# shionhonda/gae-dgl

Hardware: AMD Instinct MI355X
Metric: edges aggregated/sec (SpMM fwd+bwd) (higher is better)
Workload: dtype f32 (storage, aggregations, accumulators; the dense products run on the 16-bit matrix pipe from split operands with fp32 accumulation: X W^T and dW from three bf16 pieces per operand / six pairs, the loss from two fp16 pieces (N >= 5120) or three bf16 pieces -- all fp32-grade, see ms_per_step_exact_

## Files before the change

gae_dgl_amd/csrc/common.h:

```cpp
#pragma once
#include <hip/hip_runtime.h>
#include <stdint.h>
#include <stdio.h>

#include <atomic>

#include "gae_hip.h"
#include "gae_hip_experimental.h"

namespace gae {

struct Knob {
    std::atomic<int> v;
    explicit constexpr Knob(int x) : v(x) {}
    operator int() const { return v.load(std::memory_order_relaxed); }
    Knob &operator=(int x) { v.store(x, std::memory_order_relaxed); return *this; }
};

extern Knob g_spmm_variant, g_spmm_rpg, g_spmm_tile_vecs, g_spmm_ell, g_spmm_ell_rpg, g_spmm_hot, g_spmm_desc, g_spmm_light;
extern Knob g_gemm_rows, g_linear_wlds, g_atb_bf16, g_ell_side;
extern Knob g_xw_rows, g_xw_parts, g_xw_glds, g_xw_p3;
extern Knob g_bce_s_bf16, g_bce_pv_bf16, g_bce_sym, g_bce_sym_ri, g_bce_sym_bal, g_bce_last_kind;
extern Knob g_topk_splits, g_rank_splits;

// ... 38 lines not shown
    const unsigned xcd = bid % kNumXcd, k = bid / kNumXcd;
    const unsigned base = xcd < r ? xcd * (q + 1) : r * (q + 1) + (xcd - r) * q;
    return base + k;
}

__device__ __forceinline__ float bf16_to_f32(unsigned short v)
{
    return __uint_as_float(static_cast<unsigned>(v) << 16);
}
__device__ __forceinline__ unsigned short f32_to_bf16(float f)
{
    unsigned u = __float_as_uint(f);
    if ((u & 0x7fffffffu) > 0x7f800000u) return static_cast<unsigned short>((u >> 16) | 0x40);
    u += 0x7fffu + ((u >> 16) & 1u);
    return static_cast<unsigned short>(u >> 16);
}

typedef float v4f __attribute__((ext_vector_type(4)));
typedef float v2f __attribute__((ext_vector_type(2)));
typedef short v4s __attribute__((ext_vector_type(4)));
typedef int v4i __attribute__((ext_vector_type(4)));
typedef __bf16 v2bf __attribute__((ext_vector_type(2)));

__device__ __forceinline__ void split_bf16x4(const v4f &v, v4s &hi, v4s &lo)
{
    unsigned h[2], l[2];
#pragma unroll
    for (int q = 0; q < 2; ++q) {
        const v2f a = {v[2 * q], v[2 * q + 1]};
        const unsigned hu = __builtin_bit_cast(unsigned, __builtin_convertvector(a, v2bf));
// ... 86 lines not shown
```

gae_dgl_amd/csrc/decoder_bce.hip:

```cpp
#include <string.h>

#include "common.h"
#include "bce_finalize.h"

namespace {

using gae::kWave;
typedef float f32x4 __attribute__((ext_vector_type(4)));
typedef short s16x4 __attribute__((ext_vector_type(4)));
typedef float f32x2 __attribute__((ext_vector_type(2)));
typedef __bf16 bf16x2 __attribute__((ext_vector_type(2)));

constexpr int TJ = 64;
constexpr int PREP_ROWS = 64;
constexpr int kBceRi = 2;
constexpr int64_t kBceGrid = 2048;
constexpr int64_t kBceSymGrid = 16384;
constexpr int kChipCus = 256;
}

namespace gae {
Knob g_bce_s_bf16{3};
Knob g_bce_last_kind{0};
Knob g_bce_sym_bal{1};
// ... 43 lines not shown
    asm("v_fma_f32 %0, %1, %2, -0.5" : "=v"(s1) : "v"(r01), "v"(t[0]));
    asm("v_fma_f32 %0, %1, %2, -0.5" : "=v"(s2) : "v"(r23), "v"(t[3]));
    asm("v_fma_f32 %0, %1, %2, -0.5" : "=v"(s3) : "v"(r23), "v"(t[2]));
    return f32x4{copysignf(s0, y[0]), copysignf(s1, y[1]), copysignf(s2, y[2]), copysignf(s3, y[3])};
}

__global__ __launch_bounds__(256) void bce_prepare_kernel(const float *__restrict__ Z, float *__restrict__ mask,
                                                          int64_t ldz, int64_t n, int d, int DP, int64_t row_begin,
                                                          int64_t row_end, float *__restrict__ Zt,
                                                          unsigned short *__restrict__ Zhi,
                                                          unsigned short *__restrict__ Zlo,
                                                          double *__restrict__ colsum_partial ,
                                                          float drop_p, float drop_scale, uint64_t seed,
                                                          uint64_t offset, const uint64_t *__restrict__ draw_dev,
                                                          const int64_t *__restrict__ counts ,
                                                          double *__restrict__ scal , double all_pairs)
{
    __shared__ double red[2][256];
    const int tid = threadIdx.x;
    const int64_t n_valid = counts ? counts[0] : n;
    if (counts && blockIdx.x == 0 && tid == 0) {
        const double nv = double(counts[0]), ev = double(counts[1]);
        scal[0] = ev > 0 ? (nv * nv - ev) / ev : 0.0;
        scal[1] = nv > 0 ? 1.0 / (nv * nv) : 0.0;
        scal[2] = all_pairs - nv * nv;
    }
    const int k = tid % DP, rl = tid / DP, rpp = 256 / DP;
    const int64_t r0 = int64_t(blockIdx.x) * PREP_ROWS;
    double s_all = 0.0, s_win = 0.0;
    const bool draw = drop_p > 0.f;
    const uint64_t draw_idx = (draw && draw_dev) ? *draw_dev : 0;
    for (int rr = rl; rr < PREP_ROWS; rr += rpp) {
        const int64_t i = r0 + rr;
        if (i >= n) break;
        float v = 0.f;
        if (k < d && i >= n_valid) {
            if (draw) mask[i * ldz + k] = 0.f;
        } else if (k < d) {
            v = Z[i * ldz + k];
            if (draw) {
                const int64_t e = i * d + k;
                uint32_t c[4];
                gae::philox4x32_10(offset + uint64_t(e >> 2), draw_idx, seed, c);
                const uint32_t bits = (e & 2) ? ((e & 1) ? c[3] : c[2]) : ((e & 1) ? c[1] : c[0]);
                const float m = gae::dropout_multiplier(bits, drop_p, drop_scale);
                mask[i * ldz + k] = m;
                v *= m;
            } else if (mask) {
                v *= mask[i * ldz + k];
            }
        }
        Zt[i * DP + k] = v;
        const unsigned short hi = gae::f32_to_bf16(v);
        Zhi[i * DP + k] = hi;
        Zlo[i * DP + k] = gae::f32_to_bf16(v - gae::bf16_to_f32(hi));
        s_all += double(v);
        if (i >= row_begin && i < row_end) s_win += double(v);
    }
    red[0][tid] = s_all; red[1][tid] = s_win;
    __syncthreads();
    if (tid < DP) {
        double a = 0.0, w = 0.0;
        for (int q = 0; q < rpp; ++q) { a += red[0][q * DP + tid]; w += red[1][q * DP + tid]; }
        colsum_partial[(int64_t(blockIdx.x) * 2 + 0) * DP + tid] = a;
        colsum_partial[(int64_t(blockIdx.x) * 2 + 1) * DP + tid] = w;
    }
}

__device__ __forceinline__ void bce_colsum_block(const double *__restrict__ colsum_partial, int64_t n_blocks, int DP,
                                                 double *__restrict__ S ,
                                                 float *__restrict__ S_all_f , double *red )
{
    const int k = threadIdx.x % DP, q = threadIdx.x / DP, nq = 256 / DP;
// ... 76 lines not shown
    unsigned l2[2];
#pragma unroll
    for (int q = 0; q < 2; ++q) {
        const f32x2 a = {v[2 * q], v[2 * q + 1]};
        const f32x2 fh = {gae::bf16_to_f32((unsigned short)hi[2 * q]), gae::bf16_to_f32((unsigned short)hi[2 * q + 1])};
        const f32x2 fl = {gae::bf16_to_f32((unsigned short)lo[2 * q]), gae::bf16_to_f32((unsigned short)lo[2 * q + 1])};
        l2[q] = __builtin_bit_cast(unsigned, __builtin_convertvector((a - fh) - fl, bf16x2));
    }
    struct U { unsigned a, b; } u{l2[0], l2[1]};
    return __builtin_bit_cast(s16x4, u);
}

typedef _Float16 f16x8 __attribute__((ext_vector_type(8)));
typedef _Float16 f16x4 __attribute__((ext_vector_type(4)));
typedef __fp16 fp16x2 __attribute__((ext_vector_type(2)));
constexpr float kF16Max = 32768.f;
__device__ __forceinline__ f32x4 mfma32h(const s16x8 &a, const s16x8 &b, const f32x4 &c)
{
    return __builtin_amdgcn_mfma_f32_16x16x32_f16(__builtin_bit_cast(f16x8, a), __builtin_bit_cast(f16x8, b), c, 0, 0, 0);
}
template <bool F16>
__device__ __forceinline__ f32x4 mfma_k32(const s16x8 &a, const s16x8 &b, const f32x4 &c)
{
    if constexpr (F16) return mfma32h(a, b, c);
    else return mfma32(a, b, c);
}
typedef _Float16 f16x2 __attribute__((ext_vector_type(2)));
__device__ __forceinline__ float minus_f16_lo(float v, unsigned hh)
{
    float r;
    asm("v_fma_mix_f32 %0, %1, -1.0, %2 op_sel_hi:[1,0,0]" : "=v"(r) : "v"(hh), "v"(v));
// ... 487 lines not shown
    ew.start(Zt, DP, i, i, rowv, f0, true, wk.indptr, wk.t_indptr);
    double lsum = ew.run(Zt, DP, f0, true, pw, wk.indices, wk.t_indices);
    if (rowv) {
        f32x4 v;
#pragma unroll
        for (int q = 0; q < 4; ++q) v[q] = ew.acc_in[q] + ew.acc_out[q];
        *reinterpret_cast<f32x4 *>(wk.s + i * DP + f0) = v;
    }
#pragma unroll
    for (int off = 32; off > 0; off >>= 1) lsum += __shfl_down(lsum, off, 64);
    if (lane == 0) red[wave][0] = lsum;
    __syncthreads();
    if (tid == 0) wk.loss_partial[w] = (red[0][0] + red[1][0]) + (red[2][0] + red[3][0]);
}

enum class SymForm { kF16, kBf16x3, kBf16x3Fallback };

template <bool WITH_GRAD, int RI, SymForm FORM, bool BAL>
__global__ __launch_bounds__(256, (RI == 2 && FORM != SymForm::kBf16x3Fallback) ? 3 : 2) void bce_dense_sym_kernel(
    const float *__restrict__ Zt , const unsigned short *__restrict__ Zhi,
    const unsigned short *__restrict__ Zlo, int64_t n, int64_t cols_per_chunk,
    float *__restrict__ O_partial , float *__restrict__ Wmir,
    double *__restrict__ loss_partial , const double *__restrict__ colsum_partial,
    int64_t n_prep_blocks, double *__restrict__ S, float *__restrict__ S_all_f, unsigned n_panels, int exp_strip,
    unsigned *__restrict__ range_flag, int flag_mode, unsigned ticket, unsigned n_chunks, int bal_tpb,
    const SymWalkArgs wk)
{
    if (flag_mode == 2 && *range_flag != ticket) return;
    constexpr bool F16 = FORM == SymForm::kF16;
    constexpr bool PERSIST = FORM == SymForm::kBf16x3Fallback;
    bool out_of_range = false;
    constexpr int DP = 16, SYM_PR = 64 * RI;
    constexpr int LDH = DP + 4;
    constexpr int V4 = TJ * DP / 4 / 256;
    constexpr int LDM = TJ + 4;
    constexpr int LDHL = 2 * DP + 8;
    __shared__ __attribute__((aligned(16))) unsigned short HLs[2][TJ * LDHL];
    __shared__ __attribute__((aligned(16))) unsigned short L2s[2][F16 ? 4 : TJ * LDH];
    __shared__ __attribute__((aligned(16))) float MR[2][4][16 * LDM];
    __shared__ double red[4][2];

  double sumA = 0.0, sumL = 0.0;
  auto unit = [&](const int64_t I, const int64_t col_begin, const int64_t col_end, const int64_t op_slot, const int64_t lp_index) {
    const int tid = threadIdx.x, lane = tid & 63, wave = tid >> 6;
    const int l15 = lane & 15, g = lane >> 4;
    const int64_t NP = (n + 63) / 64 * 64;
    const int64_t row_base = SYM_PR * I + wave * (RI * 16);
    const int64_t diag_end = SYM_PR * (I + 1);

    constexpr float LOG2E = 1.44269504088896341f;
    static_assert(RI % 2 == 0, "row subtiles are paired into K = 32 mirror products");
    s16x8 bhh[RI];
    s16x8 bll[RI];
    s16x8 b3[F16 ? 1 : RI];
    s16x8 zTh[RI / 2], zTl[RI / 2];
#pragma unroll
    for (int ri = 0; ri < RI; ++ri) {
        const int64_t i = row_base + ri * 16 + l15;
        f32x4 b = *reinterpret_cast<const f32x4 *>(Zt + (i < n ? i : 0) * DP + 4 * g);
        if (i >= n) b = f32x4{0.f, 0.f, 0.f, 0.f};
        b *= LOG2E;
        s16x4 bhi, blo, blo2;
        if (F16) {
            out_of_range |= !(fmaxf(fmaxf(fabsf(b[0]), fabsf(b[1])), fmaxf(fabsf(b[2]), fabsf(b[3]))) <= kF16Max * LOG2E);
            split_f16x4(b, bhi, blo);
        } else {
            split_bf16x4_3(b, bhi, blo, blo2);
            b3[ri] = cat(bhi, blo2);
        }
        bhh[ri] = cat(bhi, bhi);
        bll[ri] = cat(blo, blo);
        s16x4 th, tl;
#pragma unroll
        for (int r = 0; r < 4; ++r) {
            const int64_t ir = row_base + ri * 16 + 4 * g + r;
            const bool v = ir < n;
            if (F16) continue;
            th[r] = v ? short(Zhi[(v ? ir : 0) * DP + l15]) : short(0);
            tl[r] = v ? short(Zlo[(v ? ir : 0) * DP + l15]) : short(0);
// ... 37 lines not shown
            const int jj = idx / (DP / 4), kk = (idx % (DP / 4)) * 4;
            const bool jv = j0 + jj < col_end;
            const int64_t j = jv ? j0 + jj : col_begin;
            st.f[q] = *reinterpret_cast<const f32x4 *>(Zt + j * DP + kk);
            if (!jv) st.f[q] = f32x4{0.f, 0.f, 0.f, 0.f};
        }
    };
    auto store_tile = [&](int buf, const Stage &st) {
#pragma unroll
        for (int q = 0; q < V4; ++q) {
            const int idx = tid + 256 * q;
            const int jj = idx / (DP / 4), kk = (idx % (DP / 4)) * 4;
            s16x4 h4, l4;
            if (F16) {
                const f32x4 f = st.f[q];
                out_of_range |= !(fmaxf(fmaxf(fabsf(f[0]), fabsf(f[1])), fmaxf(fabsf(f[2]), fabsf(f[3]))) <= kF16Max);
                split_f16x4(f, h4, l4);
            } else {
                s16x4 l24;
                split_bf16x4_3(st.f[q], h4, l4, l24);
                *reinterpret_cast<s16x4 *>(&L2s[buf][jj * LDH + kk]) = l24;
            }
            *reinterpret_cast<s16x8 *>(&HLs[buf][jj * LDHL + 2 * kk]) = cat(h4, l4);
        }
    };
    float *strip = Wmir + sym_strip_offset(I, NP, SYM_PR);
    auto flush_mirror = [&](int64_t j0, int mb) {
        const int f = tid >> 4, jq = (tid & 15) * 4;
        f32x4 v = *reinterpret_cast<const f32x4 *>(&MR[mb][0][f * LDM + jq]);
#pragma unroll
        for (int w = 1; w < 4; ++w) v += *reinterpret_cast<const f32x4 *>(&MR[mb][w][f * LDM + jq]);
// ... 106 lines not shown
        compute_tile(buf, j0, offdiag);
        if (more) store_tile(buf ^ 1, stage);
        __syncthreads();
        if (WITH_GRAD && offdiag) flush_mirror(j0, buf);
    }
    if (WITH_GRAD) {
        float *op = O_partial + op_slot * n * DP;
#pragma unroll
        for (int ri = 0; ri < RI; ++ri)
#pragma unroll
            for (int r = 0; r < 4; ++r) {
                const int64_t i = row_base + ri * 16 + 4 * g + r;
                if (i < n) op[i * DP + l15] = oacc[ri][r];
            }
    }
    if (F16 && flag_mode == 1 && out_of_range) atomicExch(range_flag, ticket);
    if (BAL) return;
    double la = sumA * 0.69314718055994531, ll = sumL;
#pragma unroll
    for (int off = 32; off > 0; off >>= 1) { la += __shfl_down(la, off, 64); ll += __shfl_down(ll, off, 64); }
    if (lane == 0) { red[wave][0] = la; red[wave][1] = ll; }
    __syncthreads();
    if (tid == 0) {
        loss_partial[2 * lp_index + 0] = (red[0][0] + red[1][0]) + (red[2][0] + red[3][0]);
        loss_partial[2 * lp_index + 1] = (red[0][1] + red[1][1]) + (red[2][1] + red[3][1]);
    }
  };
  auto unit_xy = [&](const unsigned bx, const unsigned by) {
    if (bx >= n_panels) {
        if (by == 0)
            bce_colsum_block(colsum_partial, n_prep_blocks, DP, S, S_all_f, reinterpret_cast<double *>(&MR[0][0][0]));
        return;
    }
    const int64_t col_begin = SYM_PR * int64_t(bx) + int64_t(by) * cols_per_chunk;
    const int64_t lp_index = int64_t(by) * n_panels + bx;
    if (col_begin >= n) {
        if (threadIdx.x == 0) { loss_partial[2 * lp_index] = 0.0; loss_partial[2 * lp_index + 1] = 0.0; }
        return;
    }
    const int64_t ce = col_begin + cols_per_chunk;
    unit(bx, col_begin, ce > n ? n : ce, by, lp_index);
  };
    if constexpr (BAL) {
        const unsigned n_vb = n_chunks;
        auto vblock = [&](const unsigned vb) {
        if (vb + 1 == n_vb) {
            bce_colsum_block(colsum_partial, n_prep_blocks, DP, S, S_all_f, reinterpret_cast<double *>(&MR[0][0][0]));
            return;
        }
        sumA = 0.0; sumL = 0.0;
        constexpr int TPP = SYM_PR / 64;
        const int NT = int((n + 63) / 64), T = int(n_panels);
        auto prefix = [&](int I) { return I * NT - TPP * (I * (I - 1) / 2); };
        const int W = prefix(T);
        int t0 = int(vb) * bal_tpb, t1 = t0 + bal_tpb;
        if (t1 > W) t1 = W;
        if (t0 < t1) {
            const float hb = float(NT) + 0.5f * float(TPP);
            int I = int((hb - sqrtf(fmaxf(hb * hb - 2.0f * float(TPP) * float(t0), 0.0f))) / float(TPP));
            if (I < 0) I = 0;
            if (I > T - 1) I = T - 1;
            I = __builtin_amdgcn_readfirstlane(I);
            while (I > 0 && prefix(I) > t0) --I;
            while (I + 1 < T && prefix(I + 1) <= t0) ++I;
// ... 8 lines not shown
                if (cb < n) unit(I, cb, ce, int(vb) - int(unsigned(pI) / unsigned(bal_tpb)), -1);
                __syncthreads();
                t0 += cnt; ++I;
            }
        }
        const int tid = threadIdx.x, lane = tid & 63, wave = tid >> 6;
        double la = sumA * 0.69314718055994531, ll = sumL;
#pragma unroll
        for (int off = 32; off > 0; off >>= 1) { la += __shfl_down(la, off, 64); ll += __shfl_down(ll, off, 64); }
        if (lane == 0) { red[wave][0] = la; red[wave][1] = ll; }
        __syncthreads();
        if (tid == 0) {
            loss_partial[2 * vb + 0] = (red[0][0] + red[1][0]) + (red[2][0] + red[3][0]);
            loss_partial[2 * vb + 1] = (red[0][1] + red[1][1]) + (red[2][1] + red[3][1]);
        }
        };
        if constexpr (PERSIST) {
            for (unsigned vb = blockIdx.x; vb < n_vb; vb += gridDim.x) {
                vblock(vb);
                __syncthreads();
            }
        } else if (WITH_GRAD && blockIdx.x >= n_vb) {
            const unsigned w = blockIdx.x - n_vb;
            if (w < wk.n_walk) sym_walk_block(Zt, n, w, wk, red);
        } else {
            vblock(blockIdx.x);
        }
    } else if constexpr (PERSIST) {
        const unsigned nx = n_panels + 1, total = nx * n_chunks;
        for (unsigned u = blockIdx.x; u < total; u += gridDim.x) {
            unit_xy(u % nx, u / nx);
            __syncthreads();
        }
    } else {
        unit_xy(blockIdx.x, blockIdx.y);
    }
}

__global__ __launch_bounds__(256) void bce_mirror_reduce_kernel(const float *__restrict__ Wmir, int64_t n,
                                                               float *__restrict__ Omir , int SYM_PR)
{
    const int64_t NP = (n + 63) / 64 * 64;
    const int64_t j0 = int64_t(blockIdx.x) * TJ;
    const int f = threadIdx.x >> 4, jq = (threadIdx.x & 15) * 4;
    const int64_t n_left = j0 / SYM_PR;
    f32x4 acc = {0.f, 0.f, 0.f, 0.f};
    auto at = [&](int64_t I) {
        const int64_t de = SYM_PR * (I + 1);
        return *reinterpret_cast<const f32x4 *>(Wmir + sym_strip_offset(I, NP, SYM_PR) + (j0 - de) * 16 + f * TJ + jq);
    };
// ... 322 lines not shown

extern "C" int64_t gae_decoder_bce_workspace_bytes(int64_t n, int64_t n_local, int64_t d)
{
    if (n < 0 || d < 0 || n_local < 0 || n_local > n) return GAE_E_SIZE;
    BcePlan p;
    if (!bce_plan(n, n_local, d, p)) return GAE_E_RANGE;
    return p.total_bytes + 256;
}

namespace {
inline double bce_all_pairs(const BcePlan &p, int64_t n, int64_t n_local)
{
    return p.sym ? double(n) * double(n) : double(n_local) * double((n + TJ - 1) / TJ * TJ);
}

thread_local gae_bce_tail *t_tail_out = nullptr;

int decoder_bce_impl(const float *Z, float *mask, int64_t ldz, int64_t n, int64_t d,
                     int64_t row_begin, int64_t n_local, const int32_t *indptr,
                     const int32_t *indices, const int32_t *t_indptr, const int32_t *t_indices,
                     float pos_weight, float dropout_p, uint64_t seed, uint64_t offset,
                     uint64_t *draw_dev, float *loss_out, float *dZ, int64_t lddz, void *workspace,
                     int64_t workspace_bytes, const int64_t *counts, void *stream, int64_t prepared_blocks = -1)
{
    const bool prepared = prepared_blocks >= 0;
    GAE_REQUIRE(dropout_p >= 0.f && dropout_p < 1.f, GAE_E_RANGE, "gae_decoder_bce: dropout_p = %g outside [0, 1)",
                double(dropout_p));
    GAE_REQUIRE(dropout_p == 0.f || mask, GAE_E_NULL, "gae_decoder_bce: dropout_p > 0 needs the mask output buffer");
    GAE_REQUIRE(n > 0 && d > 0, GAE_E_SIZE, "gae_decoder_bce: n and d must be positive");
    GAE_REQUIRE(row_begin >= 0 && n_local >= 0 && row_begin + n_local <= n, GAE_E_SIZE,
// ... 11 lines not shown
    if (prepared) {
        GAE_REQUIRE(prepared_blocks >= 1 && prepared_blocks * 2 * p.DP * 8 <= p.cs_bytes, GAE_E_RANGE,
                    "gae_x_decoder_bce_prepared: %lld column-sum partials do not fit the workspace", (long long)prepared_blocks);
        p.prep_blocks = prepared_blocks;
    }
    GAE_REQUIRE(gae::aligned16(workspace), GAE_E_ALIGN, "gae_decoder_bce: workspace not 16-byte aligned");
    hipStream_t s = gae::as_stream(stream);
    char *w = static_cast<char *>(workspace);
    float *O = reinterpret_cast<float *>(w); w += p.o_bytes;
    float *Zt = reinterpret_cast<float *>(w); w += p.zt_bytes;
    unsigned short *Zhi = reinterpret_cast<unsigned short *>(w); w += p.zh_bytes;
    unsigned short *Zlo = reinterpret_cast<unsigned short *>(w); w += p.zh_bytes;
    double *cs = reinterpret_cast<double *>(w); w += p.cs_bytes;
    double *S = reinterpret_cast<double *>(w);
    float *S_all_f = reinterpret_cast<float *>(w + 2 * p.DP * 8);
    double *scal = counts ? reinterpret_cast<double *>(w + 2 * p.DP * 8 + ((p.DP * 4 + 7) & ~7)) : nullptr;
    unsigned *range_flag = reinterpret_cast<unsigned *>(w + 2 * p.DP * 8 + ((p.DP * 4 + 7) & ~7) + 3 * 8);
    w += p.s_bytes;
    double *lp = reinterpret_cast<double *>(w); w += align256((2 * p.n_dense + p.edge_blocks) * 8);
    float *Wmir = reinterpret_cast<float *>(w); w += p.wmir_bytes;
    float *Omir = reinterpret_cast<float *>(w); w += p.omir_bytes;
    float *s_walk = reinterpret_cast<float *>(w);
    const double inv_n2 = 1.0 / (double(n) * double(n));
    if (n_local == 0) {
        GAE_HIP(hipMemsetAsync(loss_out, 0, sizeof(float), s));
        if (t_tail_out) { memset(t_tail_out, 0, sizeof(gae_bce_tail)); t_tail_out = nullptr; }
        return GAE_OK;
    }
    if (!prepared) {
        hipLaunchKernelGGL(bce_prepare_kernel, dim3(unsigned(p.prep_blocks)), dim3(256), 0, s, Z, mask, ldz, n, int(d), p.DP,
                           row_begin, row_begin + n_local, Zt, Zhi, Zlo, cs, dropout_p, 1.0f / (1.0f - dropout_p), seed,
                           offset, draw_dev, counts, scal, bce_all_pairs(p, n, n_local));
        GAE_CHECK_LAUNCH("bce_prepare_kernel");
    }
    int rc;
    double *lpe = lp + 2 * p.n_dense;
    const bool walk_in_dense = p.sym && p.bal_tpb && p.LPR == 4 && dZ != nullptr;
    g_bce_last_kind = p.sym ? (p.sym_pr == 256 ? 3 : 2) : 1;
    if (p.sym) {
        SymWalkArgs wk{indptr, indices, t_indptr, t_indices, pos_weight, scal, s_walk, lpe,
                       walk_in_dense ? unsigned(p.edge_blocks) : 0u};
        const dim3 grid = p.bal_tpb ? dim3(unsigned(p.bal_blocks) + 1 + wk.n_walk)
                                    : dim3(unsigned(p.row_blocks) + 1, unsigned(p.n_splits));
        static std::atomic<unsigned> call_counter{0};
        const unsigned ticket = (call_counter.fetch_add(1) * 2654435761u) | 0x80000001u;
        auto launch_sym = [&](auto kernel, dim3 g, int flag_mode) {
            hipLaunchKernelGGL(kernel, g, dim3(256), 0, s, Zt, Zhi, Zlo, n, p.cols_per_split, O, Wmir, lp, cs, p.prep_blocks, S,
                               S_all_f, unsigned(p.row_blocks), n >= 32768 ? 1 : 0, range_flag, flag_mode, ticket,
                               (p.bal_tpb ? unsigned(p.bal_blocks) + 1u : unsigned(p.n_splits)), p.bal_tpb, wk);
        };
        if (g_bce_s_bf16 == 3) {
            launch_sym(sym_kernel<SymForm::kF16>(p, dZ != nullptr), grid, 1);
            launch_sym(sym_kernel<SymForm::kBf16x3Fallback>(p, dZ != nullptr), p.bal_tpb ? dim3(64) : dim3(2 * kChipCus), 2);
        } else {
            launch_sym(sym_kernel<SymForm::kBf16x3>(p, dZ != nullptr), grid, 0);
        }
        GAE_CHECK_LAUNCH("bce_dense_sym_kernel");
        if (dZ && p.LPR != 4) {
            hipLaunchKernelGGL(bce_mirror_reduce_kernel, dim3(unsigned((n + TJ - 1) / TJ)), dim3(256), 0, s, Wmir, n,
                               Omir, p.sym_pr);
            GAE_CHECK_LAUNCH("bce_mirror_reduce_kernel");
        }
        rc = GAE_OK;
    } else {
        rc = dZ ? launch_dense<true>(p, Zt, Zhi, Zlo, n, row_begin, n_local, O, lp, cs, S, S_all_f, s)
                : launch_dense<false>(p, Zt, Zhi, Zlo, n, row_begin, n_local, O, lp, cs, S, S_all_f, s);
    }
    if (rc) return rc;
    rc = dZ ? launch_edges<true>(p, Zt, mask, ldz, row_begin, n_local, int(d), indptr, indices, t_indptr, t_indices,
                                    pos_weight, float(inv_n2), O, S_all_f, dZ, lddz, lpe, p.sym ? Omir : nullptr,
                                    counts, scal, (p.sym && p.LPR == 4) ? Wmir : nullptr,
// ... 78 lines not shown
    GAE_REQUIRE(n > 0 && d > 0 && d <= 64, GAE_E_RANGE, "gae_x_decoder_bce_prep_layout: n, d out of range");
    BcePlan p;
    bce_plan(n, n, d, p);
    GAE_REQUIRE(workspace_bytes >= p.total_bytes && gae::aligned16(workspace), GAE_E_WORKSPACE,
                "gae_x_decoder_bce_prep_layout: workspace %lld < %lld bytes (or not 16-byte aligned)",
                (long long)workspace_bytes, (long long)p.total_bytes);
    char *w = static_cast<char *>(workspace) + p.o_bytes;
    out->Zt = reinterpret_cast<float *>(w); w += p.zt_bytes;
    out->Zhi = reinterpret_cast<uint16_t *>(w); w += p.zh_bytes;
    out->Zlo = reinterpret_cast<uint16_t *>(w); w += p.zh_bytes;
    out->colsum_partial = reinterpret_cast<double *>(w); w += p.cs_bytes;
    out->scal = reinterpret_cast<double *>(w + 2 * p.DP * 8 + ((p.DP * 4 + 7) & ~7));
    out->all_pairs = bce_all_pairs(p, n, n);
    out->max_blocks = p.cs_bytes / (2 * p.DP * 8);
    out->DP = p.DP;
    out->reserved = 0;
    return GAE_OK;
}

extern "C" int gae_x_decoder_bce_prepared(float *mask, int64_t ldz, int64_t n, int64_t d, const int32_t *indptr,
                                        const int32_t *indices, const int32_t *t_indptr, const int32_t *t_indices,
                                        float pos_weight, const int64_t *counts_dev, float dropout_p,
                                        uint64_t *draw_dev, int64_t n_prep_blocks, float *loss_out, float *dZ,
                                        int64_t lddz, void *workspace, int64_t workspace_bytes, void *stream)
{
    GAE_REQUIRE(n_prep_blocks >= 1, GAE_E_RANGE, "gae_x_decoder_bce_prepared: n_prep_blocks must be what the producer reported");
    return decoder_bce_impl(nullptr, mask, ldz, n, d, 0, n, indptr, indices, t_indptr, t_indices, pos_weight, dropout_p,
                            0, 0, draw_dev, loss_out, dZ, lddz, workspace, workspace_bytes, counts_dev, stream,
                            n_prep_blocks);
}
```

gae_dgl_amd/csrc/dense.hip:

```cpp
#include <string.h>

#include "common.h"

namespace {

using gae::kWave;
typedef float f32x16 __attribute__((ext_vector_type(16)));

enum { PRO_NONE = 0, PRO_RELU_MASK = 1, PRO_MUL_MASK = 2 };
constexpr int64_t kGemmRowsMinN = 1 << 18;
}

namespace gae {
Knob g_gemm_rows{1};
Knob g_linear_wlds{1};
Knob g_atb_bf16{1};
}

namespace {
using gae::g_gemm_rows;
using gae::g_linear_wlds;
using gae::g_atb_bf16;

constexpr int BM = 128, KT = 32, LDS_LD = KT + 1;
// ... 1270 lines not shown
        const float rad = sqrtf(-2.0f * __logf(u1));
        float sn, cs;
        __sincosf(6.28318530717958648f * u2, &sn, &cs);
        z[2 * h] = rad * cs; z[2 * h + 1] = rad * sn;
    }
}

__global__ __launch_bounds__(256) void vgae_head_prep_kernel(const float *__restrict__ mu, const float *__restrict__ ls,
                                                             int64_t ldm, float *__restrict__ eps, int draw_eps,
                                                             uint64_t seed, uint64_t offset,
                                                             const uint64_t *__restrict__ draw_dev, int64_t n,
                                                             float *__restrict__ z, float *__restrict__ Zt,
                                                             unsigned short *__restrict__ Zhi,
                                                             unsigned short *__restrict__ Zlo,
                                                             double *__restrict__ colsum_partial,
                                                             double *__restrict__ kl_partial)
{
    __shared__ double red[4][17];
    const int64_t q = int64_t(blockIdx.x) * 256 + threadIdx.x;
    const int64_t i = q >> 2;
    const int k4 = int(q & 3) * 4;
    const bool in = i < n;
    float ev[4] = {0.f, 0.f, 0.f, 0.f}, zv[4] = {0.f, 0.f, 0.f, 0.f};
    double kl = 0.0;
    if (in) {
        const float4 m = *reinterpret_cast<const float4 *>(mu + i * ldm + k4);
        const float4 l = *reinterpret_cast<const float4 *>(ls + i * ldm + k4);
        if (draw_eps) {
            normal_quad(q, seed, offset, draw_dev ? *draw_dev : 0, ev);
            *reinterpret_cast<float4 *>(eps + q * 4) = make_float4(ev[0], ev[1], ev[2], ev[3]);
        } else {
            const float4 e4 = *reinterpret_cast<const float4 *>(eps + q * 4);
            ev[0] = e4.x; ev[1] = e4.y; ev[2] = e4.z; ev[3] = e4.w;
        }
        const float mm[4] = {m.x, m.y, m.z, m.w}, ll[4] = {l.x, l.y, l.z, l.w};
#pragma unroll
        for (int c = 0; c < 4; ++c) {
            const float sg = __expf(ll[c]);
            zv[c] = fmaf(ev[c], sg, mm[c]);
            kl += double(1.0f + 2.0f * ll[c] - mm[c] * mm[c] - sg * sg);
        }
        const float4 z4 = make_float4(zv[0], zv[1], zv[2], zv[3]);
        *reinterpret_cast<float4 *>(z + q * 4) = z4;
        *reinterpret_cast<float4 *>(Zt + q * 4) = z4;
        unsigned short hi[4], lo[4];
#pragma unroll
        for (int c = 0; c < 4; ++c) {
            hi[c] = gae::f32_to_bf16(zv[c]);
            lo[c] = gae::f32_to_bf16(zv[c] - gae::bf16_to_f32(hi[c]));
        }
        *reinterpret_cast<uint2 *>(Zhi + q * 4) = make_uint2(hi[0] | (unsigned(hi[1]) << 16), hi[2] | (unsigned(hi[3]) << 16));
        *reinterpret_cast<uint2 *>(Zlo + q * 4) = make_uint2(lo[0] | (unsigned(lo[1]) << 16), lo[2] | (unsigned(lo[3]) << 16));
    }
    double cs[4] = {double(zv[0]), double(zv[1]), double(zv[2]), double(zv[3])};
#pragma unroll
    for (int off = 4; off < 64; off <<= 1) {
#pragma unroll
        for (int c = 0; c < 4; ++c) cs[c] += __shfl_xor(cs[c], off, 64);
    }
// ... 285 lines not shown
    return GAE_OK;
}

extern "C" int gae_x_vgae_head_prep(const float *mu, const float *logstd, int64_t ldm, float *eps, int draw_eps,
                                  uint64_t seed, uint64_t offset, const uint64_t *draw_dev, int64_t n, int64_t d, float *z,
                                  const gae_bce_prep *prep, double *kl_partial, int64_t kl_capacity,
                                  int64_t *n_blocks_out, void *stream)
{
    GAE_REQUIRE(d == 16, GAE_E_RANGE, "gae_x_vgae_head_prep: the fused form takes d = 16 (got %lld): use gae_vgae_head_fwd", (long long)d);
    GAE_REQUIRE(n > 0 && ldm >= d && ldm % 4 == 0, GAE_E_SIZE, "gae_x_vgae_head_prep: needs n > 0 and rows of whole 16-byte vectors");
    GAE_REQUIRE(mu && logstd && eps && z && prep && kl_partial && n_blocks_out, GAE_E_NULL, "gae_x_vgae_head_prep: NULL pointer");
    GAE_REQUIRE(gae::aligned16(mu) && gae::aligned16(logstd) && gae::aligned16(eps) && gae::aligned16(z), GAE_E_ALIGN,
                "gae_x_vgae_head_prep: operands must be 16-byte aligned");
    const int64_t blocks = (n + 63) / 64;
    GAE_REQUIRE(prep->DP == 16 && blocks <= prep->max_blocks && blocks <= kl_capacity && prep->Zt && prep->Zhi &&
                    prep->Zlo && prep->colsum_partial,
                GAE_E_WORKSPACE, "gae_x_vgae_head_prep: layout / KL buffer too small for %lld blocks", (long long)blocks);
    *n_blocks_out = blocks;
    hipLaunchKernelGGL(vgae_head_prep_kernel, dim3(unsigned(blocks)), dim3(256), 0, gae::as_stream(stream), mu, logstd, ldm,
                       eps, draw_eps, seed, offset, draw_dev, n, z, prep->Zt, prep->Zhi, prep->Zlo, prep->colsum_partial,
                       kl_partial);
    GAE_CHECK_LAUNCH("vgae_head_prep_kernel");
    return GAE_OK;
}

extern "C" int gae_vgae_head_bwd(const float *dz, const float *mu, const float *logstd, int64_t ldm, const float *eps,
                                 const float *gkl_dev, int64_t n, int64_t d, float *dmu, float *dlogstd, void *stream)
{
    GAE_REQUIRE(n > 0 && d > 0 && ldm >= d && d < (1 << 24), GAE_E_SIZE, "gae_vgae_head_bwd: needs n, d > 0 and ldm >= d");
    GAE_REQUIRE(mu && logstd && eps && dmu && dlogstd, GAE_E_NULL, "gae_vgae_head_bwd: NULL pointer");
    hipLaunchKernelGGL(vgae_head_bwd_kernel, dim3(vgae_blocks(n * d)), dim3(256), 0, gae::as_stream(stream), dz, mu,
                       logstd, eps, gkl_dev, float(1.0 / (double(n) * double(n))), n * d, dmu, dlogstd, ldm, int(d));
    GAE_CHECK_LAUNCH("vgae_head_bwd_kernel");
    return GAE_OK;
}
```

gae_dgl_amd/csrc/spmm_ell.hip:

```cpp
#include <string.h>

#include <utility>

#include "common.h"

namespace {

typedef unsigned u32x4 __attribute__((ext_vector_type(4)));
typedef float f32x4 __attribute__((ext_vector_type(4)));

constexpr int32_t kEllOverflow = -2;
constexpr int32_t kEllSkip = -3;

template <int CTRL, int BANK>
__device__ __forceinline__ unsigned dpp_mov(unsigned old, unsigned v)
{
    return unsigned(__builtin_amdgcn_update_dpp(int(old), int(v), CTRL, 0xF, BANK, false));
}

template <int LP16, int K>
__device__ __forceinline__ unsigned bcast_slot(unsigned v)
{
    constexpr int ROW_NEWBCAST = 0x150;
    if constexpr (LP16 == 16) {
// ... 100 lines not shown
    int w_split, w_t;
    const float *sw_P, *sw_Q;
    float *sw_part;
    int64_t sw_ldp, sw_ldq, sw_stride;
    int sw_O, sw_I, sw_variant;
    float *pz_t;
    unsigned short *pz_hi, *pz_lo;
    double *pz_cs, *pz_scal;
    float *pz_mask;
    int64_t pz_ldmask;
    float pz_drop_p, pz_drop_scale;
    uint64_t pz_seed, pz_offset;
    const uint64_t *pz_draw;
    const int64_t *pz_counts;
    double pz_all_pairs;
};

template <typename T>
__device__ __forceinline__ void store16(T *p, const u32x4 w, int mode)
{
    if (mode == 2) {
        asm volatile("global_store_dwordx4 %0, %1, off sc1\n\ts_nop 1" ::"v"(p), "v"(w) : "memory");
    } else if (mode == 1) {
        __builtin_nontemporal_store(w, reinterpret_cast<u32x4 *>(p));
    } else {
        *reinterpret_cast<u32x4 *>(p) = w;
    }
}
__device__ __forceinline__ void store_elem(float *p, float v) { *p = v; }
__device__ __forceinline__ void store_elem(unsigned short *p, float v) { *p = gae::f32_to_bf16(v); }
// ... 218 lines not shown

    constexpr int SW_ROWS = 256 / LPR;
    constexpr int SWP = EPI_J > 0 ? SW_ROWS * 32 / 256 : 1, SWQ = EPI_J > 0 ? SW_ROWS * 64 / 256 : 1;
    __shared__ float SwP[EPI_J > 0 ? SW_ROWS * 32 : 1], SwQ[EPI_J > 0 ? SW_ROWS * 64 : 1];
    float swp[SWP], swq[SWQ];
    constexpr int JPL_K = EPI_J > 0 ? EPI_J / LPR : 1;
    int64_t pz_n_valid = a.n_rows;
    uint64_t pz_draw_idx = 0;
    if constexpr (EPI_J == 16) {
        if (a.pz_t != nullptr) {
            if (a.pz_counts) pz_n_valid = a.pz_counts[0];
            if (a.pz_drop_p > 0.f && a.pz_draw) pz_draw_idx = *a.pz_draw;
        }
    }
    double pz_sum[JPL_K];
    float pz_m[JPL_K];
#pragma unroll
    for (int q = 0; q < JPL_K; ++q) pz_m[q] = 1.f;
#pragma unroll
    for (int q = 0; q < JPL_K; ++q) pz_sum[q] = 0.0;
    constexpr int SW_K = EPI_J > 0 ? SW_ROWS / 4 : 1;
    float sda[SW_K], sdb[SW_K];
    bool sw_direct = false;
    int sd_mt = 0, sd_nt = 0;
    bool sd_ones = false, sd_live = false;
    if constexpr (EPI_J > 0) {
        if (a.sw_part != nullptr && (a.sw_variant & 8)) {
            const int mt_n = (a.sw_O + 15) >> 4, nt_n = (a.sw_I + 15) >> 4;
            sw_direct = mt_n * nt_n + mt_n <= 4;
            if (sw_direct) {
// ... 204 lines not shown
                        if (a.act == GAE_ACT_RELU) y = fmaxf(y, 0.f);
                        a.Y[row[r] * a.ldy + o] = y;
                        yv[q] = y;
                    }
                }
            }
            if constexpr (EPI_J == 16) {
                if (a.pz_t != nullptr) {
                    const bool in = row[r] < a.n_rows;
#pragma unroll
                    for (int q = 0; q < JPL; ++q) {
                        const int o = lig * JPL + q;
                        const float v = (in && o < a.J) ? yv[q] * pz_m[q] : 0.f;
                        if (in) {
                            a.pz_t[row[r] * 16 + o] = v;
                            const unsigned short hi = gae::f32_to_bf16(v);
                            a.pz_hi[row[r] * 16 + o] = hi;
                            a.pz_lo[row[r] * 16 + o] = gae::f32_to_bf16(v - gae::bf16_to_f32(hi));
                        }
                        pz_sum[q] = double(v);
                    }
                }
            }
        }
    }
    if constexpr (EPI_J == 16) {
        if (a.pz_t != nullptr) {
            double *cred = reinterpret_cast<double *>(SwQ);
#pragma unroll
            for (int q = 0; q < JPL_K; ++q) {
#pragma unroll
                for (int off = LPR; off < 64; off <<= 1) pz_sum[q] += __shfl_xor(pz_sum[q], off, 64);
                if ((threadIdx.x & 63) < LPR) cred[(threadIdx.x >> 6) * 16 + lig * JPL_K + q] = pz_sum[q];
            }
            __syncthreads();
            if (threadIdx.x < 16) {
                const double t = ((cred[threadIdx.x] + cred[16 + threadIdx.x]) + cred[32 + threadIdx.x]) + cred[48 + threadIdx.x];
                a.pz_cs[(int64_t(blk) * 2 + 0) * 16 + threadIdx.x] = t;
                a.pz_cs[(int64_t(blk) * 2 + 1) * 16 + threadIdx.x] = t;
            }
            if (a.pz_counts && blk == 0 && threadIdx.x == 0) {
                const double nv = double(a.pz_counts[0]), ev = double(a.pz_counts[1]);
// ... 243 lines not shown
    a.empty_off = a.h_bytes; a.n_splits = 1;
    a.n_cols = unsigned(n_cols); a.F = unsigned(F); a.nvec = unsigned((F + 3) / 4);
    a.tile_vecs = a.nvec;
    a.xcd_tiled = 0; a.store_pad = 0; a.store_mode = 0;
    a.W = W; a.bias = bias; a.Y = Y; a.ldy = ldy; a.J = int(J); a.w_so = int(w_stride_out); a.w_sk = int(w_stride_in);
    a.act = act; a.store_m = M != nullptr;
    a.W2 = W2; a.bias2 = bias2; a.w_split = int(w_split); a.w_t = w_transposed;
    if (side) {
        a.sw_P = side->P; a.sw_Q = side->Q; a.sw_part = side->part;
        a.sw_ldp = side->ldp; a.sw_ldq = side->ldq; a.sw_stride = side->stride; a.sw_O = side->O; a.sw_I = side->I;
        a.sw_variant = int(gae::g_ell_side);
    }
    if (prep) {
        a.pz_t = prep->lay->Zt; a.pz_hi = prep->lay->Zhi; a.pz_lo = prep->lay->Zlo; a.pz_cs = prep->lay->colsum_partial;
        a.pz_scal = prep->lay->scal; a.pz_all_pairs = prep->lay->all_pairs;
        a.pz_mask = prep->mask; a.pz_ldmask = prep->ldmask; a.pz_drop_p = prep->drop_p;
        a.pz_drop_scale = 1.0f / (1.0f - prep->drop_p);
        a.pz_seed = prep->seed; a.pz_offset = prep->offset; a.pz_draw = prep->draw; a.pz_counts = prep->counts;
    }
    hipStream_t s = gae::as_stream(stream);
    const bool scaled = row_scale != nullptr;
    const int ew = plan->ell_width;
    if (a.nvec <= 8) return J <= 16 ? launch_ell_epi_w<8, 16>(a, ew, scaled, s) : launch_ell_epi_w<8, 32>(a, ew, scaled, s);
    return J <= 16 ? launch_ell_epi_w<16, 16>(a, ew, scaled, s) : launch_ell_epi_w<16, 32>(a, ew, scaled, s);
}

extern "C" int gae_x_gcn_layer_fused_prep(const int32_t *indptr, const int32_t *indices, int64_t n, const float *H,
                                        int64_t ldh, float *M, int64_t ldm, int64_t F, const float *row_scale,
                                        const float *col_scale, const gae_spmm_plan *plan, const float *W,
                                        int64_t w_stride_out, int64_t w_stride_in, const float *bias, int64_t J,
                                        float *Z, int64_t ldz, const gae_bce_prep *prep, float *mask, int64_t ldmask,
                                        float dropout_p, uint64_t seed, uint64_t offset, const uint64_t *draw_dev,
                                        const int64_t *counts_dev, int64_t *n_prep_blocks_out, void *stream)
{
    GAE_REQUIRE(prep && n_prep_blocks_out, GAE_E_NULL, "gae_x_gcn_layer_fused_prep: NULL pointer");
    GAE_REQUIRE(J >= 1 && J <= 16 && prep->DP == 16, GAE_E_RANGE,
                "gae_x_gcn_layer_fused_prep: the embedding must be at most 16 wide (got %lld)", (long long)J);
    GAE_REQUIRE(dropout_p >= 0.f && dropout_p < 1.f, GAE_E_RANGE, "gae_x_gcn_layer_fused_prep: dropout_p outside [0, 1)");
    GAE_REQUIRE(dropout_p == 0.f || mask, GAE_E_NULL, "gae_x_gcn_layer_fused_prep: dropout_p > 0 needs the mask output buffer");
    GAE_REQUIRE(!mask || ldmask >= J, GAE_E_SIZE, "gae_x_gcn_layer_fused_prep: ldmask < J");
    GAE_REQUIRE(n >= 1, GAE_E_SIZE, "gae_x_gcn_layer_fused_prep: empty graph");
    const int64_t rpb = (F + 3) / 4 <= 8 ? 32 : 16, blocks = (n + rpb - 1) / rpb;
    GAE_REQUIRE(blocks <= prep->max_blocks && prep->Zt && prep->Zhi && prep->Zlo && prep->colsum_partial, GAE_E_WORKSPACE,
                "gae_x_gcn_layer_fused_prep: layout not from gae_x_decoder_bce_prep_layout for this n");
    *n_prep_blocks_out = blocks;
    FusedPrep fp{prep, mask, ldmask, dropout_p, seed, offset, draw_dev, counts_dev};
    return gcn_layer_fused_impl(indptr, indices, n, n, H, ldh, M, ldm, F, row_scale, col_scale, plan, W, w_stride_out,
                                w_stride_in, bias, J, GAE_ACT_IDENTITY, Z, ldz, nullptr, nullptr, 0, 0, stream, nullptr, &fp);
}

static int64_t fused_wgrad_blocks(int64_t n_rows, int64_t F) { const int64_t rpb = (F + 3) / 4 <= 8 ? 32 : 16; return (n_rows + rpb - 1) / rpb; }

extern "C" int64_t gae_x_gcn_layer_fused_wgrad_workspace_bytes(int64_t n_rows, int64_t F, int64_t I)
{
    if (n_rows < 0 || F < 1 || F > 32 || I < 1 || I > 64) return GAE_E_SIZE;
    return fused_wgrad_blocks(n_rows, F) * (F * I + F) * 4 + 256;
}

// ... 125 lines not shown
```

Baseline: 1.341 billion.

## Detect fp16 range overflow in prep kernels and drop the fallback BCE relaunch

```diff
diff --git a/gae_dgl_amd/csrc/common.h b/gae_dgl_amd/csrc/common.h
--- a/gae_dgl_amd/csrc/common.h
+++ b/gae_dgl_amd/csrc/common.h
@@ -76,6 +76,13 @@
     if ((u & 0x7fffffffu) > 0x7f800000u) return static_cast<unsigned short>((u >> 16) | 0x40);
     u += 0x7fffu + ((u >> 16) & 1u);
     return static_cast<unsigned short>(u >> 16);
+}
+
+constexpr float kBceF16Max = 32768.f;
+__device__ __forceinline__ bool bce_f16_out_of_range(float z)
+{
+    constexpr float LOG2E = 1.44269504088896341f;
+    return !(fabsf(z) <= kBceF16Max) || !(fabsf(z * LOG2E) <= kBceF16Max * LOG2E);
 }
 
 typedef float v4f __attribute__((ext_vector_type(4)));
diff --git a/gae_dgl_amd/csrc/decoder_bce.hip b/gae_dgl_amd/csrc/decoder_bce.hip
--- a/gae_dgl_amd/csrc/decoder_bce.hip
+++ b/gae_dgl_amd/csrc/decoder_bce.hip
@@ -1,4 +1,8 @@
 #include <string.h>
+#include <atomic>
+#include <mutex>
+#include <type_traits>
+#include <unordered_map>
 
 #include "common.h"
 #include "bce_finalize.h"
@@ -81,7 +85,8 @@
                                                           float drop_p, float drop_scale, uint64_t seed,
                                                           uint64_t offset, const uint64_t *__restrict__ draw_dev,
                                                           const int64_t *__restrict__ counts ,
-                                                          double *__restrict__ scal , double all_pairs)
+                                                          double *__restrict__ scal , double all_pairs,
+                                                          unsigned *__restrict__ range_flag, unsigned ticket)
 {
     __shared__ double red[2][256];
     const int tid = threadIdx.x;
@@ -97,6 +102,7 @@
     double s_all = 0.0, s_win = 0.0;
     const bool draw = drop_p > 0.f;
     const uint64_t draw_idx = (draw && draw_dev) ? *draw_dev : 0;
+    bool out_of_range = false;
     for (int rr = rl; rr < PREP_ROWS; rr += rpp) {
         const int64_t i = r0 + rr;
         if (i >= n) break;
@@ -118,12 +124,14 @@
             }
         }
         Zt[i * DP + k] = v;
+        out_of_range |= gae::bce_f16_out_of_range(v);
         const unsigned short hi = gae::f32_to_bf16(v);
         Zhi[i * DP + k] = hi;
         Zlo[i * DP + k] = gae::f32_to_bf16(v - gae::bf16_to_f32(hi));
         s_all += double(v);
         if (i >= row_begin && i < row_end) s_win += double(v);
     }
+    if (out_of_range) atomicExch(range_flag, ticket);
     red[0][tid] = s_all; red[1][tid] = s_win;
     __syncthreads();
     if (tid < DP) {
@@ -230,7 +238,7 @@
 typedef _Float16 f16x8 __attribute__((ext_vector_type(8)));
 typedef _Float16 f16x4 __attribute__((ext_vector_type(4)));
 typedef __fp16 fp16x2 __attribute__((ext_vector_type(2)));
-constexpr float kF16Max = 32768.f;
+constexpr float kF16Max = gae::kBceF16Max;
 __device__ __forceinline__ f32x4 mfma32h(const s16x8 &a, const s16x8 &b, const f32x4 &c)
 {
     return __builtin_amdgcn_mfma_f32_16x16x32_f16(__builtin_bit_cast(f16x8, a), __builtin_bit_cast(f16x8, b), c, 0, 0, 0);
@@ -748,33 +756,48 @@
     if (tid == 0) wk.loss_partial[w] = (red[0][0] + red[1][0]) + (red[2][0] + red[3][0]);
 }
 
-enum class SymForm { kF16, kBf16x3, kBf16x3Fallback };
+enum class SymForm { kF16, kBf16x3 };
+
+constexpr int kSymLdh = 16 + 4;
+constexpr int kSymLdm = TJ + 4;
+constexpr int kSymLdhl = 2 * 16 + 8;
 
 template <bool WITH_GRAD, int RI, SymForm FORM, bool BAL>
-__global__ __launch_bounds__(256, (RI == 2 && FORM != SymForm::kBf16x3Fallback) ? 3 : 2) void bce_dense_sym_kernel(
+__global__ __launch_bounds__(256, RI == 2 ? 3 : 2) void bce_dense_sym_kernel(
     const float *__restrict__ Zt , const unsigned short *__restrict__ Zhi,
     const unsigned short *__restrict__ Zlo, int64_t n, int64_t cols_per_chunk,
     float *__restrict__ O_partial , float *__restrict__ Wmir,
     double *__restrict__ loss_partial , const double *__restrict__ colsum_partial,
     int64_t n_prep_blocks, double *__restrict__ S, float *__restrict__ S_all_f, unsigned n_panels, int exp_strip,
-    unsigned *__restrict__ range_flag, int flag_mode, unsigned ticket, unsigned n_chunks, int bal_tpb,
-    const SymWalkArgs wk)
-{
-    if (flag_mode == 2 && *range_flag != ticket) return;
-    constexpr bool F16 = FORM == SymForm::kF16;
-    constexpr bool PERSIST = FORM == SymForm::kBf16x3Fallback;
-    bool out_of_range = false;
+    const unsigned *__restrict__ range_flag, unsigned ticket, unsigned n_chunks, int bal_tpb, const SymWalkArgs wk)
+{
     constexpr int DP = 16, SYM_PR = 64 * RI;
-    constexpr int LDH = DP + 4;
+    constexpr int LDH = kSymLdh, LDM = kSymLdm, LDHL = kSymLdhl;
     constexpr int V4 = TJ * DP / 4 / 256;
-    constexpr int LDM = TJ + 4;
-    constexpr int LDHL = 2 * DP + 8;
     __shared__ __attribute__((aligned(16))) unsigned short HLs[2][TJ * LDHL];
-    __shared__ __attribute__((aligned(16))) unsigned short L2s[2][F16 ? 4 : TJ * LDH];
+    __shared__ __attribute__((aligned(16))) unsigned short L2s[2][TJ * LDH];
     __shared__ __attribute__((aligned(16))) float MR[2][4][16 * LDM];
     __shared__ double red[4][2];
 
-  double sumA = 0.0, sumL = 0.0;
+    if constexpr (BAL) {
+        if (WITH_GRAD && blockIdx.x >= n_chunks) {
+            const unsigned w = blockIdx.x - n_chunks;
+            if (w < wk.n_walk) sym_walk_block(Zt, n, w, wk, red);
+            return;
+        }
+        if (blockIdx.x + 1 == n_chunks) {
+            bce_colsum_block(colsum_partial, n_prep_blocks, DP, S, S_all_f, reinterpret_cast<double *>(&MR[0][0][0]));
+            return;
+        }
+    } else if (blockIdx.x >= n_panels) {
+        if (blockIdx.y == 0)
+            bce_colsum_block(colsum_partial, n_prep_blocks, DP, S, S_all_f, reinterpret_cast<double *>(&MR[0][0][0]));
+        return;
+    }
+
+  auto body = [&](auto f16_tag) __attribute__((always_inline)) {
+    constexpr bool F16 = decltype(f16_tag)::value;
+    double sumA = 0.0, sumL = 0.0;
   auto unit = [&](const int64_t I, const int64_t col_begin, const int64_t col_end, const int64_t op_slot, const int64_t lp_index) {
     const int tid = threadIdx.x, lane = tid & 63, wave = tid >> 6;
     const int l15 = lane & 15, g = lane >> 4;
@@ -796,7 +819,6 @@
         b *= LOG2E;
         s16x4 bhi, blo, blo2;
         if (F16) {
-            out_of_range |= !(fmaxf(fmaxf(fabsf(b[0]), fabsf(b[1])), fmaxf(fabsf(b[2]), fabsf(b[3]))) <= kF16Max * LOG2E);
             split_f16x4(b, bhi, blo);
         } else {
             split_bf16x4_3(b, bhi, blo, blo2);
@@ -864,7 +886,6 @@
             s16x4 h4, l4;
             if (F16) {
                 const f32x4 f = st.f[q];
-                out_of_range |= !(fmaxf(fmaxf(fabsf(f[0]), fabsf(f[1])), fmaxf(fabsf(f[2]), fabsf(f[3]))) <= kF16Max);
                 split_f16x4(f, h4, l4);
             } else {
                 s16x4 l24;
@@ -1001,7 +1022,6 @@
                 if (i < n) op[i * DP + l15] = oacc[ri][r];
             }
     }
-    if (F16 && flag_mode == 1 && out_of_range) atomicExch(range_flag, ticket);
     if (BAL) return;
     double la = sumA * 0.69314718055994531, ll = sumL;
 #pragma unroll
@@ -1013,28 +1033,8 @@
         loss_partial[2 * lp_index + 1] = (red[0][1] + red[1][1]) + (red[2][1] + red[3][1]);
     }
   };
-  auto unit_xy = [&](const unsigned bx, const unsigned by) {
-    if (bx >= n_panels) {
-        if (by == 0)
-            bce_colsum_block(colsum_partial, n_prep_blocks, DP, S, S_all_f, reinterpret_cast<double *>(&MR[0][0][0]));
-        return;
-    }
-    const int64_t col_begin = SYM_PR * int64_t(bx) + int64_t(by) * cols_per_chunk;
-    const int64_t lp_index = int64_t(by) * n_panels + bx;
-    if (col_begin >= n) {
-        if (threadIdx.x == 0) { loss_partial[2 * lp_index] = 0.0; loss_partial[2 * lp_index + 1] = 0.0; }
-        return;
-    }
-    const int64_t ce = col_begin + cols_per_chunk;
-    unit(bx, col_begin, ce > n ? n : ce, by, lp_index);
-  };
     if constexpr (BAL) {
-        const unsigned n_vb = n_chunks;
-        auto vblock = [&](const unsigned vb) {
-        if (vb + 1 == n_vb) {
-            bce_colsum_block(colsum_partial, n_prep_blocks, DP, S, S_all_f, reinterpret_cast<double *>(&MR[0][0][0]));
-            return;
-        }
+        const unsigned vb = blockIdx.x;
         sumA = 0.0; sumL = 0.0;
         constexpr int TPP = SYM_PR / 64;
         const int NT = int((n + 63) / 64), T = int(n_panels);
@@ -1073,26 +1073,23 @@
             loss_partial[2 * vb + 0] = (red[0][0] + red[1][0]) + (red[2][0] + red[3][0]);
             loss_partial[2 * vb + 1] = (red[0][1] + red[1][1]) + (red[2][1] + red[3][1]);
         }
-        };
-        if constexpr (PERSIST) {
-            for (unsigned vb = blockIdx.x; vb < n_vb; vb += gridDim.x) {
-                vblock(vb);
-                __syncthreads();
-            }
-        } else if (WITH_GRAD && blockIdx.x >= n_vb) {
-            const unsigned w = blockIdx.x - n_vb;
-            if (w < wk.n_walk) sym_walk_block(Zt, n, w, wk, red);
-        } else {
-            vblock(blockIdx.x);
-        }
-    } else if constexpr (PERSIST) {
-        const unsigned nx = n_panels + 1, total = nx * n_chunks;
-        for (unsigned u = blockIdx.x; u < total; u += gridDim.x) {
-            unit_xy(u % nx, u / nx);
-            __syncthreads();
-        }
     } else {
-        unit_xy(blockIdx.x, blockIdx.y);
+        const unsigned bx = blockIdx.x, by = blockIdx.y;
+        const int64_t col_begin = SYM_PR * int64_t(bx) + int64_t(by) * cols_per_chunk;
+        const int64_t lp_index = int64_t(by) * n_panels + bx;
+        if (col_begin >= n) {
+            if (threadIdx.x == 0) { loss_partial[2 * lp_index] = 0.0; loss_partial[2 * lp_index + 1] = 0.0; }
+            return;
+        }
+        const int64_t ce = col_begin + cols_per_chunk;
+        unit(bx, col_begin, ce > n ? n : ce, by, lp_index);
+    }
+  };
+    if constexpr (FORM == SymForm::kF16) {
+        if (*range_flag == ticket) body(std::false_type{});
+        else body(std::true_type{});
+    } else {
+        body(std::false_type{});
     }
 }
 
@@ -1445,6 +1442,15 @@
     return p.sym ? double(n) * double(n) : double(n_local) * double((n + TJ - 1) / TJ * TJ);
 }
 
+unsigned bce_new_ticket()
+{
+    static std::atomic<unsigned> call_counter{0};
+    return (call_counter.fetch_add(1) * 2654435761u) | 0x80000001u;
+}
+std::mutex g_prep_ticket_mutex;
+std::unordered_map<const void *, unsigned> g_prep_tickets;
+inline unsigned *bce_range_flag(double *scal) { return reinterpret_cast<unsigned *>(scal + 3); }
+
 thread_local gae_bce_tail *t_tail_out = nullptr;
 
 int decoder_bce_impl(const float *Z, float *mask, int64_t ldz, int64_t n, int64_t d,
@@ -1486,8 +1492,9 @@
     double *cs = reinterpret_cast<double *>(w); w += p.cs_bytes;
     double *S = reinterpret_cast<double *>(w);
     float *S_all_f = reinterpret_cast<float *>(w + 2 * p.DP * 8);
-    double *scal = counts ? reinterpret_cast<double *>(w + 2 * p.DP * 8 + ((p.DP * 4 + 7) & ~7)) : nullptr;
-    unsigned *range_flag = reinterpret_cast<unsigned *>(w + 2 * p.DP * 8 + ((p.DP * 4 + 7) & ~7) + 3 * 8);
+    double *scal_slots = reinterpret_cast<double *>(w + 2 * p.DP * 8 + ((p.DP * 4 + 7) & ~7));
+    double *scal = counts ? scal_slots : nullptr;
+    unsigned *range_flag = bce_range_flag(scal_slots);
     w += p.s_bytes;
     double *lp = reinterpret_cast<double *>(w); w += align256((2 * p.n_dense + p.edge_blocks) * 8);
     float *Wmir = reinterpret_cast<float *>(w); w += p.wmir_bytes;
@@ -1499,10 +1506,20 @@
         if (t_tail_out) { memset(t_tail_out, 0, sizeof(gae_bce_tail)); t_tail_out = nullptr; }
         return GAE_OK;
     }
+    unsigned ticket;
+    if (prepared) {
+        std::lock_guard<std::mutex> lock(g_prep_ticket_mutex);
+        const auto it = g_prep_tickets.find(workspace);
+        GAE_REQUIRE(it != g_prep_tickets.end(), GAE_E_WORKSPACE,
+                    "gae_x_decoder_bce_prepared: no gae_x_decoder_bce_prep_layout call for this workspace");
+        ticket = it->second;
+    } else {
+        ticket = bce_new_ticket();
+    }
     if (!prepared) {
         hipLaunchKernelGGL(bce_prepare_kernel, dim3(unsigned(p.prep_blocks)), dim3(256), 0, s, Z, mask, ldz, n, int(d), p.DP,
                            row_begin, row_begin + n_local, Zt, Zhi, Zlo, cs, dropout_p, 1.0f / (1.0f - dropout_p), seed,
-                           offset, draw_dev, counts, scal, bce_all_pairs(p, n, n_local));
+                           offset, draw_dev, counts, scal, bce_all_pairs(p, n, n_local), range_flag, ticket);
         GAE_CHECK_LAUNCH("bce_prepare_kernel");
     }
     int rc;
@@ -1514,19 +1531,13 @@
                        walk_in_dense ? unsigned(p.edge_blocks) : 0u};
         const dim3 grid = p.bal_tpb ? dim3(unsigned(p.bal_blocks) + 1 + wk.n_walk)
                                     : dim3(unsigned(p.row_blocks) + 1, unsigned(p.n_splits));
-        static std::atomic<unsigned> call_counter{0};
-        const unsigned ticket = (call_counter.fetch_add(1) * 2654435761u) | 0x80000001u;
-        auto launch_sym = [&](auto kernel, dim3 g, int flag_mode) {
-            hipLaunchKernelGGL(kernel, g, dim3(256), 0, s, Zt, Zhi, Zlo, n, p.cols_per_split, O, Wmir, lp, cs, p.prep_blocks, S,
-                               S_all_f, unsigned(p.row_blocks), n >= 32768 ? 1 : 0, range_flag, flag_mode, ticket,
+        auto launch_sym = [&](auto kernel) {
+            hipLaunchKernelGGL(kernel, grid, dim3(256), 0, s, Zt, Zhi, Zlo, n, p.cols_per_split, O, Wmir, lp, cs, p.prep_blocks,
+                               S, S_all_f, unsigned(p.row_blocks), n >= 32768 ? 1 : 0, range_flag, ticket,
                                (p.bal_tpb ? unsigned(p.bal_blocks) + 1u : unsigned(p.n_splits)), p.bal_tpb, wk);
         };
-        if (g_bce_s_bf16 == 3) {
-            launch_sym(sym_kernel<SymForm::kF16>(p, dZ != nullptr), grid, 1);
-            launch_sym(sym_kernel<SymForm::kBf16x3Fallback>(p, dZ != nullptr), p.bal_tpb ? dim3(64) : dim3(2 * kChipCus), 2);
-        } else {
-            launch_sym(sym_kernel<SymForm::kBf16x3>(p, dZ != nullptr), grid, 0);
-        }
+        if (g_bce_s_bf16 == 3) launch_sym(sym_kernel<SymForm::kF16>(p, dZ != nullptr));
+        else launch_sym(sym_kernel<SymForm::kBf16x3>(p, dZ != nullptr));
         GAE_CHECK_LAUNCH("bce_dense_sym_kernel");
         if (dZ && p.LPR != 4) {
             hipLaunchKernelGGL(bce_mirror_reduce_kernel, dim3(unsigned((n + TJ - 1) / TJ)), dim3(256), 0, s, Wmir, n,
@@ -1635,7 +1646,12 @@
     out->all_pairs = bce_all_pairs(p, n, n);
     out->max_blocks = p.cs_bytes / (2 * p.DP * 8);
     out->DP = p.DP;
-    out->reserved = 0;
+    const unsigned ticket = bce_new_ticket();
+    out->reserved = int32_t(ticket);
+    {
+        std::lock_guard<std::mutex> lock(g_prep_ticket_mutex);
+        g_prep_tickets[workspace] = ticket;
+    }
     return GAE_OK;
 }
 
diff --git a/gae_dgl_amd/csrc/dense.hip b/gae_dgl_amd/csrc/dense.hip
--- a/gae_dgl_amd/csrc/dense.hip
+++ b/gae_dgl_amd/csrc/dense.hip
@@ -1308,7 +1308,8 @@
                                                              unsigned short *__restrict__ Zhi,
                                                              unsigned short *__restrict__ Zlo,
                                                              double *__restrict__ colsum_partial,
-                                                             double *__restrict__ kl_partial)
+                                                             double *__restrict__ kl_partial,
+                                                             unsigned *__restrict__ range_flag, unsigned ticket)
 {
     __shared__ double red[4][17];
     const int64_t q = int64_t(blockIdx.x) * 256 + threadIdx.x;
@@ -1337,6 +1338,9 @@
         const float4 z4 = make_float4(zv[0], zv[1], zv[2], zv[3]);
         *reinterpret_cast<float4 *>(z + q * 4) = z4;
         *reinterpret_cast<float4 *>(Zt + q * 4) = z4;
+        if (gae::bce_f16_out_of_range(zv[0]) | gae::bce_f16_out_of_range(zv[1]) | gae::bce_f16_out_of_range(zv[2]) |
+            gae::bce_f16_out_of_range(zv[3]))
+            atomicExch(range_flag, ticket);
         unsigned short hi[4], lo[4];
 #pragma unroll
         for (int c = 0; c < 4; ++c) {
@@ -1652,12 +1656,12 @@
                 "gae_x_vgae_head_prep: operands must be 16-byte aligned");
     const int64_t blocks = (n + 63) / 64;
     GAE_REQUIRE(prep->DP == 16 && blocks <= prep->max_blocks && blocks <= kl_capacity && prep->Zt && prep->Zhi &&
-                    prep->Zlo && prep->colsum_partial,
+                    prep->Zlo && prep->colsum_partial && prep->scal && prep->reserved != 0,
                 GAE_E_WORKSPACE, "gae_x_vgae_head_prep: layout / KL buffer too small for %lld blocks", (long long)blocks);
     *n_blocks_out = blocks;
     hipLaunchKernelGGL(vgae_head_prep_kernel, dim3(unsigned(blocks)), dim3(256), 0, gae::as_stream(stream), mu, logstd, ldm,
                        eps, draw_eps, seed, offset, draw_dev, n, z, prep->Zt, prep->Zhi, prep->Zlo, prep->colsum_partial,
-                       kl_partial);
+                       kl_partial, reinterpret_cast<unsigned *>(prep->scal + 3), unsigned(prep->reserved));
     GAE_CHECK_LAUNCH("vgae_head_prep_kernel");
     return GAE_OK;
 }
diff --git a/gae_dgl_amd/csrc/spmm_ell.hip b/gae_dgl_amd/csrc/spmm_ell.hip
--- a/gae_dgl_amd/csrc/spmm_ell.hip
+++ b/gae_dgl_amd/csrc/spmm_ell.hip
@@ -138,6 +138,8 @@
     const uint64_t *pz_draw;
     const int64_t *pz_counts;
     double pz_all_pairs;
+    unsigned *pz_flag;
+    unsigned pz_ticket;
 };
 
 template <typename T>
@@ -386,6 +388,7 @@
         }
     }
     double pz_sum[JPL_K];
+    bool pz_oor = false;
     float pz_m[JPL_K];
 #pragma unroll
     for (int q = 0; q < JPL_K; ++q) pz_m[q] = 1.f;
@@ -620,6 +623,7 @@
                         const float v = (in && o < a.J) ? yv[q] * pz_m[q] : 0.f;
                         if (in) {
                             a.pz_t[row[r] * 16 + o] = v;
+                            pz_oor |= gae::bce_f16_out_of_range(v);
                             const unsigned short hi = gae::f32_to_bf16(v);
                             a.pz_hi[row[r] * 16 + o] = hi;
                             a.pz_lo[row[r] * 16 + o] = gae::f32_to_bf16(v - gae::bf16_to_f32(hi));
@@ -632,6 +636,7 @@
     }
     if constexpr (EPI_J == 16) {
         if (a.pz_t != nullptr) {
+            if (pz_oor) atomicExch(a.pz_flag, a.pz_ticket);
             double *cred = reinterpret_cast<double *>(SwQ);
 #pragma unroll
             for (int q = 0; q < JPL_K; ++q) {
@@ -905,6 +910,8 @@
     if (prep) {
         a.pz_t = prep->lay->Zt; a.pz_hi = prep->lay->Zhi; a.pz_lo = prep->lay->Zlo; a.pz_cs = prep->lay->colsum_partial;
         a.pz_scal = prep->lay->scal; a.pz_all_pairs = prep->lay->all_pairs;
+        a.pz_flag = reinterpret_cast<unsigned *>(prep->lay->scal + 3);
+        a.pz_ticket = unsigned(prep->lay->reserved);
         a.pz_mask = prep->mask; a.pz_ldmask = prep->ldmask; a.pz_drop_p = prep->drop_p;
         a.pz_drop_scale = 1.0f / (1.0f - prep->drop_p);
         a.pz_seed = prep->seed; a.pz_offset = prep->offset; a.pz_draw = prep->draw; a.pz_counts = prep->counts;
@@ -932,7 +939,9 @@
     GAE_REQUIRE(!mask || ldmask >= J, GAE_E_SIZE, "gae_x_gcn_layer_fused_prep: ldmask < J");
     GAE_REQUIRE(n >= 1, GAE_E_SIZE, "gae_x_gcn_layer_fused_prep: empty graph");
     const int64_t rpb = (F + 3) / 4 <= 8 ? 32 : 16, blocks = (n + rpb - 1) / rpb;
-    GAE_REQUIRE(blocks <= prep->max_blocks && prep->Zt && prep->Zhi && prep->Zlo && prep->colsum_partial, GAE_E_WORKSPACE,
+    GAE_REQUIRE(blocks <= prep->max_blocks && prep->Zt && prep->Zhi && prep->Zlo && prep->colsum_partial && prep->scal &&
+                    prep->reserved != 0,
+                GAE_E_WORKSPACE,
                 "gae_x_gcn_layer_fused_prep: layout not from gae_x_decoder_bce_prep_layout for this n");
     *n_prep_blocks_out = blocks;
     FusedPrep fp{prep, mask, ldmask, dropout_p, seed, offset, draw_dev, counts_dev};
```

After: 1.354 billion (median of 6 runs). No clear change (+0.9%).
